# EmbersArc/SCpp

Measured on AMD Instinct MI355X. Metric: converged SCvx trajectories/sec (RocketQuat, K=50) at 1/2/4/8 MI355X, higher is better.
Workload: dtype f64

## Files before the change

### scpp_amd/csrc/common.h

```cpp
#pragma once
#ifdef SCPP_HIP_EMU
#include "hip_emu.h"
#else
#include <hip/hip_runtime.h>
typedef double d4_t __attribute__((ext_vector_type(4)));
#endif
#include <cmath>
#include <cstdint>

namespace scpp
{

constexpr int WAVE = 64;

#ifdef SCPP_HIP_EMU
#define WAVE_SYNC() __syncthreads()
#else
#define WAVE_SYNC()                                            \
    do                                                         \
    {                                                          \
        __builtin_amdgcn_fence(__ATOMIC_ACQ_REL, "wavefront"); \
        __builtin_amdgcn_wave_barrier();                       \
    } while (0)
#endif
// ... 190 lines not shown
__host__ __device__ inline Dual1 dsqrt(Dual1 a)
{
    const double r = sqrt(a.v);
    return Dual1(r, a.d * 0.5 / r);
}
__host__ __device__ inline Dual1 dsin(Dual1 a) { return Dual1(sin(a.v), a.d * cos(a.v)); }
__host__ __device__ inline Dual1 dcos(Dual1 a) { return Dual1(cos(a.v), -a.d * sin(a.v)); }
__host__ __device__ inline double dsqrt(double a) { return sqrt(a); }
__host__ __device__ inline double dsin(double a) { return sin(a); }
__host__ __device__ inline double dcos(double a) { return cos(a); }
__host__ __device__ inline double valueOf(double a) { return a; }
__host__ __device__ inline double valueOf(Dual1 a) { return a.v; }
__host__ __device__ inline double tangentOf(double) { return 0.; }
__host__ __device__ inline double tangentOf(Dual1 a) { return a.d; }

constexpr int RK_S = 13;
constexpr double RK_C[RK_S] = {0., 2. / 27., 1. / 9., 1. / 6., 5. / 12., 1. / 2., 5. / 6., 1. / 6., 2. / 3., 1. / 3., 1., 0., 1.};
constexpr double RK_A[RK_S][RK_S] = {
    {0},
    {2. / 27.},
    {1. / 36., 1. / 12.},
    {1. / 24., 0., 1. / 8.},
    {5. / 12., 0., -25. / 16., 25. / 16.},
    {1. / 20., 0., 0., 1. / 4., 1. / 5.},
    {-25. / 108., 0., 0., 125. / 108., -65. / 27., 125. / 54.},
    {31. / 300., 0., 0., 0., 61. / 225., -2. / 9., 13. / 900.},
    {2., 0., 0., -53. / 6., 704. / 45., -107. / 9., 67. / 90., 3.},
    {-91. / 108., 0., 0., 23. / 108., -976. / 135., 311. / 54., -19. / 60., 17. / 6., -1. / 12.},
    {2383. / 4100., 0., 0., -341. / 164., 4496. / 1025., -301. / 82., 2133. / 4100., 45. / 82., 45. / 164., 18. / 41.},
    {3. / 205., 0., 0., 0., 0., -6. / 41., -3. / 205., -3. / 41., 3. / 41., 6. / 41., 0.},
    {-1777. / 4100., 0., 0., -341. / 164., 4496. / 1025., -289. / 82., 2193. / 4100., 51. / 82., 33. / 164., 12. / 41., 0., 1.}};
constexpr double RK_B[RK_S] = {0., 0., 0., 0., 0., 34. / 105., 9. / 35., 9. / 35., 9. / 280., 9. / 280., 0., 41. / 840., 41. / 840.};

}
```

### scpp_amd/csrc/discretize_kernel.h

```cpp
#pragma once
#include "common.h"
#include <utility>

namespace scpp
{

template <class F, int... S>
__device__ inline void forEachStageImpl(F &&f, std::integer_sequence<int, S...>)
{
    (f(std::integral_constant<int, S>{}), ...);
}
template <class F>
__device__ inline void forEachStage(F &&f)
{
    forEachStageImpl(f, std::make_integer_sequence<int, RK_S>{});
}

#ifndef DISC_STEPS
#define DISC_STEPS 0
#endif
#ifndef DISC_MAX_STEP
#define DISC_MAX_STEP (12. / (14. * 5.))
#endif
constexpr int DISC_STEPS_MAX = 5;
#ifndef DISC_WAVES_PER_SIMD
#define DISC_WAVES_PER_SIMD 2
#endif

template <class Model, bool FOH, bool VT>
struct DiscLayout
{
    static constexpr int NX = Model::NX, NU = Model::NU, NP = Model::NP;
    static constexpr int NJ = NX + NU;
    static constexpr int NCOLS = 1 + NX + NU + (FOH ? NU : 0) + (VT ? 1 : 0);
    static constexpr int NENT = NX * NCOLS;
    static constexpr int NG = WAVE / 16;
    static constexpr int EPL = (NCOLS + NG - 1) / NG;
    static constexpr int COL_S = 1, COL_PHI = 1 + (VT ? 1 : 0), COL_B = COL_PHI + NX, COL_C = COL_B + NU;
    static constexpr int NJP = (NJ + 1) & ~1;
};

template <class Model, bool FOH, bool VT>
struct DiscLds
{
    using L = DiscLayout<Model, FOH, VT>;
    __attribute__((aligned(16))) double Ys[32 * L::NX + 2];
#ifdef DISC_AD_JACOBIAN
    __attribute__((aligned(16))) double Jm[L::NX * L::NJP];
    double fv[L::NX];
    double cst[L::NP + 2 * L::NU + 1];
#else
    double uh[DISC_STEPS_MAX * RK_S * (Model::JacobianRows::NUAUX + 1 + L::NU)];
    __attribute__((aligned(16))) double Wt[Model::JacobianTable::NW];
    double cst[L::NP + 2 * L::NU + Model::JacobianRows::NAUX + 1];
#endif
};

template <class Model, bool FOH, bool VT>
__device__ __forceinline__ void discretizeSegment(int B, int K, const double *__restrict__ X, const double *__restrict__ U,
                                                  const double *__restrict__ sigma, const double *__restrict__ par, int par_stride,
                                                  const int *__restrict__ active, double *__restrict__ Aout, double *__restrict__ Bout,
                                                  double *__restrict__ Cout, double *__restrict__ Sout, double *__restrict__ Zout, int steps_opt,
                                                  const long inst, const int k, DiscLds<Model, FOH, VT> *lds)
{
    using L = DiscLayout<Model, FOH, VT>;
    constexpr int NX = L::NX, NU = L::NU, NP = L::NP, NJ = L::NJ, NJP = L::NJP, NCOLS = L::NCOLS, NG = L::NG, EPL = L::EPL;

    static_assert(NX <= 16 && NCOLS + NG <= 32 && NG == 4, "one 16-row tile of states, two 16-column tiles of V");
    auto &Ys = lds->Ys;
#ifndef DISC_AD_JACOBIAN
    constexpr int NAUX = Model::JacobianRows::NAUX;
    constexpr int NUAUX = Model::JacobianRows::NUAUX;
    constexpr int UHP = NUAUX + 1 + NU;
    auto &uh = lds->uh;
#define DISC_TABLE_ROWS 1
    using TB = typename Model::JacobianTable;
    auto &Wt = lds->Wt;
#else
    constexpr int NAUX = 0;
    auto &Jm = lds->Jm;
    auto &fv = lds->fv;
#endif
    auto &cst = lds->cst;

    const int lane = threadIdx.x;
    for (int i = lane; i < 32 * NX + 2; i += WAVE)
        Ys[i] = 0.;
    const int nseg = K - 1;
    if (inst >= B)
        return;
    if (active && active[inst] == 0)
// ... 99 lines not shown
    const int row = lane & 15, g = lane >> 4;
    const bool lane_on = row < NX;
#ifndef SCPP_HIP_EMU
    __builtin_assume(g >= 0 && g < NG);
#endif
    const double x0r = lane_on ? X[(inst * K + k) * NX + row] : 0.;
    double y[EPL];
    bool eon[EPL];
#pragma unroll
    for (int m = 0; m < EPL; m++)
    {
        const int c = m * NG + g;
        eon[m] = lane_on && c < NCOLS;
        double v = 0.;
        if (c == 0)
            v = x0r;
        else if (c >= L::COL_PHI && c < L::COL_PHI + NX)
            v = (c - L::COL_PHI == row) ? 1. : 0.;
        y[m] = eon[m] ? v : 0.;
    }

    double kk[RK_S][EPL];
    const double h = dt / double(nsteps);
#ifdef DISC_PROFILE
    long long tA = 0, tB = 0, tC = 0;
    const long long tk0 = clock64();
#endif

    for (int step = 0; step < nsteps; step++)
    {
        const double t0 = double(step) * h;
        forEachStage([&](auto sc) {
            constexpr int s = decltype(sc)::value;
#ifdef DISC_PROFILE
            const long long p0 = clock64();
#endif
            const double ts = t0 + RK_C[s] * h;
#pragma unroll
            for (int m = 0; m < EPL; m++)
            {
                double acc = 0.;
#pragma unroll
                for (int j = 0; j < s; j++)
                    if (RK_A[s][j] != 0.)
                        acc += RK_A[s][j] * kk[j][m];
                const double ys = y[m] + h * acc;
                if (eon[m])
                    Ys[(m * NG + g) * NX + row] = ys;
#ifdef DISC_TABLE_ROWS
                if (m == 0 && g == 0 && lane_on)
                    Wt[TB::W_X + row] = ys;
#endif
            }
            WAVE_SYNC();
#ifdef DISC_PROFILE
            const long long p1 = clock64();
            tA += p1 - p0;
#endif
#ifndef DISC_AD_JACOBIAN
            const double frac = FOH ? uh[(step * RK_S + s) * UHP + NUAUX] : 0.;
#else
            const double frac = FOH ? ts / dt : 0.;
#endif
            double jr[NJ];
            double fr;
#ifdef DISC_TABLE_ROWS
// ... 200 lines not shown
            continue;
        Ys[c * NX + row] = y[m];
        if (c >= L::COL_PHI && c < L::COL_PHI + NX)
            Aout[seg * NX * NX + row * NX + (c - L::COL_PHI)] = y[m];
        else if (c >= L::COL_B && c < L::COL_B + NU)
            Bout[seg * NX * NU + row * NU + (c - L::COL_B)] = y[m];
        else if (FOH && c >= L::COL_C && c < L::COL_C + NU)
            Cout[seg * NX * NU + row * NU + (c - L::COL_C)] = y[m];
        else if (VT && c == L::COL_S)
            Sout[seg * NX + row] = y[m];
    }
    if (lane < NX)
        Ys[NCOLS * NX + lane] = x0r;
    WAVE_SYNC();
    if (lane < NX)
    {
        double z = Ys[lane];
#pragma unroll
        for (int j = 0; j < NX; j++)
            z -= Ys[(L::COL_PHI + j) * NX + lane] * Ys[NCOLS * NX + j];
#pragma unroll
        for (int j = 0; j < NU; j++)
        {
            z -= Ys[(L::COL_B + j) * NX + lane] * u0[j];
            if (FOH)
                z -= Ys[(L::COL_C + j) * NX + lane] * u1[j];
        }
        if (VT)
            z -= Ys[L::COL_S * NX + lane] * sg;
        Zout[seg * NX + lane] = z;
    }
}

template <class Model, bool FOH, bool VT>
__global__ void __launch_bounds__(WAVE, DISC_WAVES_PER_SIMD)
    discretize_kernel(int B, int K, const double *__restrict__ X, const double *__restrict__ U,
                      const double *__restrict__ sigma, const double *__restrict__ par, int par_stride,
                      const int *__restrict__ active,
                      double *__restrict__ Aout, double *__restrict__ Bout, double *__restrict__ Cout,
                      double *__restrict__ Sout, double *__restrict__ Zout, int steps_opt)
{
    const int nseg = K - 1;
    const long b = blockIdx.x;
    const long xcd = b & 7, gb = b >> 3;
    const long inst = (gb / nseg) * 8 + xcd;
    const int k = int(gb % nseg);
    __shared__ DiscLds<Model, FOH, VT> lds;
    discretizeSegment<Model, FOH, VT>(B, K, X, U, sigma, par, par_stride, active, Aout, Bout, Cout, Sout, Zout, steps_opt, inst, k, &lds);
}

template <class Model>
__global__ void simulate_kernel(int B, const double *__restrict__ par, int par_stride, const double *__restrict__ dtv,
                                const double *__restrict__ u0v, const double *__restrict__ u1v, double *__restrict__ x,
                                const int *__restrict__ active)
{
    constexpr int NX = Model::NX, NU = Model::NU, NP = Model::NP;
    const long i = long(blockIdx.x) * blockDim.x + threadIdx.x;
    if (i >= B)
        return;
    if (active && active[i] == 0)
        return;
    double p[NP], u0[NU], u1[NU], y[NX], kk[RK_S][NX];
    for (int j = 0; j < NP; j++)
        p[j] = par[i * par_stride + j];
    for (int j = 0; j < NU; j++)
    {
        u0[j] = u0v[i * NU + j];
        u1[j] = u1v[i * NU + j];
    }
    for (int j = 0; j < NX; j++)
        y[j] = x[i * NX + j];
    const double dt = dtv[i];
    const double h = dt / 20.;
    for (int step = 0; step < 20; step++)
    {
        const double t0 = double(step) * h;
#pragma unroll
        for (int s = 0; s < RK_S; s++)
        {
            double ys[NX], u[NU];
            const double ts = t0 + RK_C[s] * h;
            for (int j = 0; j < NX; j++)
            {
                double acc = 0.;
#pragma unroll
                for (int q = 0; q < s; q++)
                    if (RK_A[s][q] != 0.)
                        acc += RK_A[s][q] * kk[q][j];
                ys[j] = y[j] + h * acc;
            }
            for (int j = 0; j < NU; j++)
                u[j] = u0[j] + ts / dt * (u1[j] - u0[j]);
            Model::template systemFlowMap<double>(ys, u, p, kk[s]);
        }
        for (int j = 0; j < NX; j++)
        {
            double acc = 0.;
#pragma unroll
            for (int s = 0; s < RK_S; s++)
                if (RK_B[s] != 0.)
                    acc += RK_B[s] * kk[s][j];
            y[j] += h * acc;
        }
    }
    for (int j = 0; j < NX; j++)
        x[i * NX + j] = y[j];
}

}
```

### scpp_amd/csrc/scpp_hip.cpp

```cpp
#include "../../include/scpp_hip.h"

#include <algorithm>
#include <cmath>
#include <utility>
#include <cstdio>
#include <cstdlib>
#include <cstring>
#include <mutex>
#include <new>
#include <tuple>
#include <vector>

#include "common.h"
#include "discretize_kernel.h"
#include "ipm_solve.h"
#include "ipm_split.h"
#include "model_rocketquat.h"
#include "sc_kernels.h"
#include "scvx_kernels.h"
#include "scvx_persistent.h"
#include "mpc_kernel.h"
#include "mpc_setup.h"

using namespace scpp;

#define CHECK_HIP(expr)                  \
    do                                   \
    {                                    \
        hipError_t e_ = (expr);          \
        if (e_ != hipSuccess)            \
            return SCPP_E_HIP;           \
    } while (0)

template <class L>
struct ParamsOf;
template <class... PL>
struct ParamsOf<PluginList<PL...>>
{
    using type = std::tuple<typename PL::Params...>;
};
template <class F, class... PL>
int withPluginOf(PluginList<PL...>, int model, F &&f)
{
// ... 40 lines not shown
    mpc::MpcConst *mpc_const = nullptr;
    mpc::MpcConst *mpc_host = nullptr;
    double *mpc_xf = nullptr, *mpc_x0 = nullptr, *mpc_U = nullptr, *mpc_X = nullptr, *mpc_cost = nullptr, *mpc_uheld = nullptr, *mpc_t = nullptr;
    int *mpc_status = nullptr, *mpc_iters = nullptr, *mpc_steps = nullptr, *mpc_failed = nullptr, *mpc_ipm = nullptr, *mpc_reached = nullptr;
    bool mpc_ready = false;
    int mpc_B = 0;
    double *sim_dt = nullptr, *sim_u0 = nullptr, *sim_u1 = nullptr, *sim_x = nullptr;
    scpp_sc_opts sc{};
    ParamsOf<Plugins>::type model_params{};
    size_t ws_per = 0;
    scpp_socp_opts socp{1e-8, 1e-7, 1e-7, 60, 1};
    bool sc_ready = false, par_from_ip = false;
    bool sc_warm = false;
    int sc_persistent_min = 3072;
    int mode = SCPP_MODE_FOH | SCPP_MODE_VT;
    struct Span
    {
        hipEvent_t a, b;
        int kind;
        long long inst;
    };
    std::vector<Span> spans;
    std::vector<hipEvent_t> pool;
    scpp_timing timing{};
    hipEvent_t ev_base = nullptr;
    int last_active = 0;
    long long stream_rounds = 0;
    int stream_pools = 0;
    int stream_engine = SCPP_STREAM_ENGINE_DEFAULT;
    double *persist_shares = nullptr;
    unsigned long long stream_ticks[4] = {0, 0, 0, 0};
    int ipm_schedule = SCPP_IPM_SCHEDULE_DEFAULT;
    int ipm_split_pairs = 0;
    int disc_steps = 5;
};

namespace
{

struct DeviceGuard
{
    int prev = -1;
    bool switched = false;
    explicit DeviceGuard(const scpp_hip_ctx *c)
    {
        if (!c)
            return;
        if (hipGetDevice(&prev) == hipSuccess && prev != c->device)
            switched = hipSetDevice(c->device) == hipSuccess;
    }
    ~DeviceGuard()
    {
        if (switched)
            (void)hipSetDevice(prev);
    }
};

template <class T>
int devAlloc(T **p, size_t n)
{
    return hipMalloc(reinterpret_cast<void **>(p), n * sizeof(T)) == hipSuccess ? 0 : -1;
}

hipEvent_t getEvent(scpp_hip_ctx *c)
{
    if (!c->pool.empty())
// ... 88 lines not shown
        else
            c->timing.ms_other += ms;
        if (s.kind == 0 || s.kind == 1)
        {
            if (based)
                iv[s.kind].emplace_back(double(t0), double(t0) + double(ms));
            else
                (s.kind == 0 ? c->timing.ms_discretize_union : c->timing.ms_socp_union) += ms;
        }
        c->pool.push_back(s.a);
        c->pool.push_back(s.b);
    }
    c->timing.ms_discretize_union += unionLength(iv[0]);
    c->timing.ms_socp_union += unionLength(iv[1]);
    c->spans.clear();
}

template <class Model>
int launchDiscretize(scpp_hip_ctx *c, int mode, const double *par0, int stride, const int *active0, long long ninst, Range r)
{
    const int B = r.count, K = c->K;
    const long groups = ((long(B) + 7) / 8) * (K - 1);
    const unsigned grid = unsigned(groups * 8);
    const size_t f = size_t(r.first), nx = size_t(c->nx), nu = size_t(c->nu), seg = size_t(K - 1);
    const double *par = par0 + f * size_t(stride);
    const int *active = active0 ? active0 + f : nullptr;
    struct
    {
        double *X, *U, *sigma, *A, *Bm, *C, *S, *Z;
        hipStream_t stream;
    } v{c->X + f * K * nx, c->U + f * K * nu, c->sigma + f, c->A + f * seg * nx * nx, c->Bm + f * seg * nx * nu,
        c->C + f * seg * nx * nu, c->S + f * seg * nx, c->Z + f * seg * nx, r.stream};
    const bool timed = spanBegin(c, 0, ninst, r.stream);
    if (mode == (SCPP_MODE_FOH | SCPP_MODE_VT))
        hipLaunchKernelGGL((discretize_kernel<Model, true, true>), dim3(grid), dim3(WAVE), 0, v.stream, B, K, v.X, v.U,
                           v.sigma, par, stride, active, v.A, v.Bm, v.C, v.S, v.Z, c->disc_steps);
    else if (mode == SCPP_MODE_FOH)
        hipLaunchKernelGGL((discretize_kernel<Model, true, false>), dim3(grid), dim3(WAVE), 0, v.stream, B, K, v.X, v.U,
                           v.sigma, par, stride, active, v.A, v.Bm, v.C, v.S, v.Z, c->disc_steps);
    else if (mode == SCPP_MODE_VT)
        hipLaunchKernelGGL((discretize_kernel<Model, false, true>), dim3(grid), dim3(WAVE), 0, v.stream, B, K, v.X, v.U,
                           v.sigma, par, stride, active, v.A, v.Bm, v.C, v.S, v.Z, c->disc_steps);
    else
        hipLaunchKernelGGL((discretize_kernel<Model, false, false>), dim3(grid), dim3(WAVE), 0, v.stream, B, K, v.X, v.U,
                           v.sigma, par, stride, active, v.A, v.Bm, v.C, v.S, v.Z, c->disc_steps);
    spanEnd(c, timed, r.stream);
    return hipGetLastError() == hipSuccess ? 0 : SCPP_E_HIP;
}

int discretizeDispatch(scpp_hip_ctx *c, int mode, const double *par, int stride, const int *active, long long ninst, Range r)
{
    return withPlugin(c->model, [&](auto pl) { return launchDiscretize<typename decltype(pl)::Model>(c, mode, par, stride, active, ninst, r); });
}
int discretizeDispatch(scpp_hip_ctx *c, int mode, const double *par, int stride, const int *active, long long ninst)
{
    return discretizeDispatch(c, mode, par, stride, active, ninst, fullRange(c));
}

SCBuffers scBuffers(scpp_hip_ctx *c)
{
    SCBuffers b;
    b.B = c->B;
    b.K = c->K;
    b.x_init_dim = c->x_init;
    b.X = c->X;
    b.U = c->U;
    b.sigma = c->sigma;
    b.ip = c->ip;
    b.uhat = c->uhat;
    b.wtrx = c->wtrx;
    b.active = c->active;
    b.converged = c->converged;
    b.sc_iters = c->sc_iters;
    b.ipm_iters = c->ipm_iters;
    b.status = c->status;
    b.norm1_nu = c->norm1_nu;
    b.sum_delta = c->sum_delta;
    b.delta_sigma = c->delta_sigma;
// ... 243 lines not shown
#if !defined(SCPP_HIP_EMU) && !SCPP_TOOLCHAIN_VALIDATED
    {
        static std::once_flag warned;
        std::call_once(warned, [] {
            std::fprintf(stderr, "scpp_hip: built with an unvalidated toolchain (%s); run `pytest -m gpu` before trusting results\n", scpp_hip_version());
        });
    }
#endif
    int prev_device = -1;
    (void)hipGetDevice(&prev_device);
    CHECK_HIP(hipSetDevice(device_id));
    struct Restore
    {
        int d;
        ~Restore()
        {
            if (d >= 0)
                (void)hipSetDevice(d);
        }
    } restore{prev_device == device_id ? -1 : prev_device};
    if (int rc = tileSelfTest(device_id))
        return rc;
    scpp_hip_ctx *c = new (std::nothrow) scpp_hip_ctx;
    if (!c)
        return SCPP_E_HIP;
    c->device = device_id;
    c->model = model_id;
    c->K = K;
    c->Bmax = batch_max;
    c->B = 0;
    if (const char *e = std::getenv("SCPP_IPM_SCHEDULE"))
        if (std::atoi(e) >= SCPP_IPM_RESIDENT && std::atoi(e) <= SCPP_IPM_SPLIT)
            c->ipm_schedule = std::atoi(e);
    if (const char *e = std::getenv("SCPP_STREAM_ENGINE"))
        if (std::atoi(e) == SCPP_STREAM_POOLS || std::atoi(e) == SCPP_STREAM_PERSISTENT)
            c->stream_engine = std::atoi(e);
    if (const char *e = std::getenv("SCPP_SC_PERSISTENT_MIN"))
        if (std::atoi(e) > 0)
            c->sc_persistent_min = std::atoi(e);
    if (const char *e = std::getenv("SCPP_IPM_SPLIT_PAIRS"))
        if (std::atoi(e) > 0)
            c->ipm_split_pairs = std::atoi(e);
    (void)withPlugin(model_id, [&](auto pl) {
        using PL = decltype(pl);
        c->nx = PL::Model::NX;
        c->nu = PL::Model::NU;
        c->np = PL::Model::NP;
        c->ws_per = ipm::workspaceDoubles<typename PL::Table>(K);
        return 0;
    });
    if (hipStreamCreate(&c->stream) != hipSuccess)
    {
        delete c;
        return SCPP_E_HIP;
    }
    const size_t B = size_t(batch_max), nx = c->nx, nu = c->nu;
    int rc = 0;
    rc |= devAlloc(&c->X, B * K * nx);
    rc |= devAlloc(&c->U, B * K * nu);
    rc |= devAlloc(&c->sigma, B);
    rc |= devAlloc(&c->par, B * c->np);
    rc |= devAlloc(&c->A, B * (K - 1) * nx * nx);
    rc |= devAlloc(&c->Bm, B * (K - 1) * nx * nu);
    rc |= devAlloc(&c->C, B * (K - 1) * nx * nu);
    rc |= devAlloc(&c->S, B * (K - 1) * nx);
    rc |= devAlloc(&c->Z, B * (K - 1) * nx);
// ... 1551 lines not shown
```

### scpp_amd/csrc/scvx_kernels.h

```cpp
#pragma once
#include "discretize_kernel.h"
#include "sc_kernels.h"

namespace scpp
{

constexpr int SCVX_SOLVE_CAP = 64;

struct SCvxBuffers
{
    double *Xold, *Uold;
    double *tr;
    double *last_cost;
    double *cost;
    double *info;
    int *has_last, *needs_disc, *solves;
    double *iter_ring;
    int *iter_count;
    int iter_cap;
};
constexpr int SCVX_ITER_SCALARS = 4;
__host__ __device__ inline size_t scvxIterRecordDoubles(int K, int nx, int nu) { return size_t(K) * size_t(nx + nu) + SCVX_ITER_SCALARS; }
__device__ inline void scvxRecordIterate(const SCBuffers &b, const SCvxBuffers &v, long i, int nx, int nu, int lane, int lanes)
{
// ... 154 lines not shown
#endif
template <class Model>
__device__ __forceinline__ void scvxCostUpdate(const SCBuffers &b, const SCvxBuffers &v, const scpp_scvx_opts &so, const long i)
{
    using namespace ipm;
    constexpr int NX = Model::NX, NU = Model::NU, NP = Model::NP;
    if (i >= b.B || b.active[i] == 0)
        return;
    const int K = b.K, k = threadIdx.x;
    const int foh = so.interpolate_input;
    double acc = 0.;
    if (k < K - 1 && b.status[i] == 0)
    {
        double p[NP], u0[NU], u1[NU], y[NX], kk[RK_S][NX];
        const double *ip = b.ip + i * IP_N;
        for (int j = 0; j < NP; j++)
            p[j] = ip[IP_PAR + j];
        const double *X = b.X + (i * K + k) * NX, *U = b.U + (i * K + k) * NU;
        for (int j = 0; j < NU; j++)
        {
            u0[j] = U[j];
            u1[j] = foh ? U[NU + j] : U[j];
        }
        for (int j = 0; j < NX; j++)
            y[j] = X[j];
        const double dt = b.sigma[i] / double(K - 1);
        const double h = dt / 20.;
        for (int step = 0; step < 20; step++)
        {
            const double t0 = double(step) * h;
#pragma unroll
            for (int s = 0; s < RK_S; s++)
            {
                double ys[NX], u[NU];
                const double ts = t0 + RK_C[s] * h;
                for (int j = 0; j < NX; j++)
                {
                    double a = 0.;
#pragma unroll
                    for (int q = 0; q < s; q++)
                        if (RK_A[s][q] != 0.)
                            a += RK_A[s][q] * kk[q][j];
                    ys[j] = y[j] + h * a;
                }
                for (int j = 0; j < NU; j++)
                    u[j] = u0[j] + ts / dt * (u1[j] - u0[j]);
                Model::template systemFlowMap<double>(ys, u, p, kk[s]);
            }
            for (int j = 0; j < NX; j++)
            {
                double a = 0.;
#pragma unroll
                for (int s = 0; s < RK_S; s++)
                    if (RK_B[s] != 0.)
                        a += RK_B[s] * kk[s][j];
                y[j] += h * a;
            }
        }
        for (int j = 0; j < NX; j++)
            acc += fabs(y[j] - X[NX + j]);
    }
    acc = wave_sum(acc);
    int flags = 0;
    if (k == 0)
    {
        v.cost[i] = acc;
// ... 28 lines not shown
    const int half = lane & 1, pair = lane >> 1;
    const bool solved = b.status[i] == 0;
    if (lane < WAVE)
        seg_sum[lane] = 0.;
    WAVE_SYNC();
    for (int pass = 0; pass * 32 < K - 1; pass++)
    {
        const int k = pass * 32 + pair;
        const bool on = k < K - 1 && solved;
        const int kc = on ? k : 0;
        double p[NP], u0[NU], u1[NU], y[NH], kk[RK_S][NH];
        const double *ip = b.ip + i * IP_N;
#pragma unroll
        for (int j = 0; j < NP; j++)
            p[j] = ip[IP_PAR + j];
        const double *X = b.X + (i * K + kc) * NX, *U = b.U + (i * K + kc) * NU;
#pragma unroll
        for (int j = 0; j < NU; j++)
        {
            u0[j] = U[j];
            u1[j] = foh ? U[NU + j] : U[j];
        }
#pragma unroll
        for (int j = 0; j < NH; j++)
            y[j] = (j < NH1 || !half) ? X[half * NH + j] : 0.;
        const double dt = b.sigma[i] / double(K - 1);
        const double h = dt / 20.;
        for (int step = 0; step < 20; step++)
        {
            const double t0 = double(step) * h;
#pragma unroll
            for (int s = 0; s < RK_S; s++)
            {
                double mine[NH], ys[NX], u[NU], f[NX];
                const double ts = t0 + RK_C[s] * h;
#pragma unroll
                for (int j = 0; j < NH; j++)
                {
                    double a = 0.;
#pragma unroll
                    for (int q = 0; q < s; q++)
                        if (RK_A[s][q] != 0.)
                            a += RK_A[s][q] * kk[q][j];
                    mine[j] = y[j] + h * a;
                }
#pragma unroll
                for (int j = 0; j < NH; j++)
                {
                    const double other = __shfl_xor(mine[j], 1);
                    ys[j] = half ? other : mine[j];
                    if (j < NH1)
                        ys[NH + j] = half ? mine[j] : other;
                }
#pragma unroll
                for (int j = 0; j < NU; j++)
                    u[j] = u0[j] + ts / dt * (u1[j] - u0[j]);
                Model::template systemFlowMap<double>(ys, u, p, f);
#pragma unroll
                for (int j = 0; j < NH; j++)
                    kk[s][j] = half ? (j < NH1 ? f[NH + j < NX ? NH + j : 0] : 0.) : f[j];
            }
#pragma unroll
            for (int j = 0; j < NH; j++)
            {
                double a = 0.;
#pragma unroll
// ... 151 lines not shown
```

### scpp_amd/csrc/scvx_persistent.h

```cpp
#pragma once
#include "discretize_kernel.h"
#include "ipm_solve.h"
#include "scvx_kernels.h"

namespace scpp
{

#ifndef PERSIST_COST_SPLIT
#define PERSIST_COST_SPLIT 1
#endif
struct PersistentOut
{
    double *A, *Bm, *C, *S, *Z;
    int disc_steps;
    double *shares;
};
template <class T>
struct PersistentArgs
{
    ipm::KernelArgs a;
    SCBuffers b;
    SCvxBuffers v;
    StreamQueue q;
    typename T::Params mp;
// ... 72 lines not shown
}
__device__ __forceinline__ int uniformLoad(const int *p)
{
    return uniformInt(*(const volatile int *)p);
}

template <class T>
PERSIST_STEP_FN void persistRefill(long slot)
{
    PERSIST_ARGS(T, A);
    const SCBuffers b = argCopy(A.b);
    const SCvxBuffers v = argCopy(A.v);
    const StreamQueue q = argCopy(A.q);
    const typename T::Params mp = argCopy(A.mp);
    const scpp_sc_opts sc = argCopy(A.sc);
    const scpp_scvx_opts so = argCopy(A.so);
    scvxStreamRefill<T>(b, v, q, mp, sc, so, slot);
    stepFence();
}
template <class T, class Model, bool FOH>
PERSIST_STEP_FN void persistDiscretize(long slot)
{
    PERSIST_ARGS(T, A);
    const int B = A.b.B, K = A.b.K, steps = A.o.disc_steps;
    const double *X = A.a.X, *U = A.a.U, *sigma = A.a.sigma, *par = A.b.ip + ipm::IP_PAR;
    double *Ao = A.o.A, *Bo = A.o.Bm, *Co = A.o.C, *So = A.o.S, *Zo = A.o.Z;
#ifdef SCPP_HIP_EMU
    static DiscLds<Model, FOH, false> lds_obj;
    DiscLds<Model, FOH, false> *lds = &lds_obj;
#else
    extern __shared__ __attribute__((aligned(16))) double seg_lds[];
    DiscLds<Model, FOH, false> *lds = reinterpret_cast<DiscLds<Model, FOH, false> *>(seg_lds);
#endif
    for (int k = 0; k < K - 1; k++)
    {
        discretizeSegment<Model, FOH, false>(B, K, X, U, sigma, par, ipm::IP_N, nullptr, Ao, Bo, Co, So, Zo, steps, slot, k, lds);
        WAVE_SYNC();
    }
    stepFence();
}
template <class T, class P>
PERSIST_STEP_FN void persistSolve(long slot)
{
    PERSIST_ARGS(T, A);
    const ipm::KernelArgs a = argCopy(A.a);
    ipm::ipmSolveInstance<P>(a, int(slot), &A.a);
    if (IPM_PRIO_LANE)
        SET_PRIO(0);
    stepFence();
}
template <class T, class Model>
PERSIST_STEP_FN void persistCost(long slot)
{
    PERSIST_ARGS(T, A);
    const SCBuffers b = argCopy(A.b);
    const SCvxBuffers v = argCopy(A.v);
    const scpp_scvx_opts so = argCopy(A.so);
#if PERSIST_COST_SPLIT
#ifdef SCPP_HIP_EMU
    static double seg_sum[WAVE];
#else
    extern __shared__ __attribute__((aligned(16))) double seg_lds[];
    double *seg_sum = seg_lds;
#endif
    scvxCostUpdateSplit<Model>(b, v, so, slot, seg_sum);
#else
    scvxCostUpdate<Model>(b, v, so, slot);
#endif
    stepFence();
}

// ... 30 lines not shown
        t_disc += t2 - t1;
        t_ipm += t3 - t2;
        t_cost += t4 - t3;
    }
#ifndef SCPP_HIP_EMU
    {
        PERSIST_ARGS(T, A);
        if (A.o.shares && threadIdx.x == 0)
        {
            unsigned long long *sh = reinterpret_cast<unsigned long long *>(A.o.shares);
            atomicAdd(sh + 0, (unsigned long long)t_ref);
            atomicAdd(sh + 1, (unsigned long long)t_disc);
            atomicAdd(sh + 2, (unsigned long long)t_ipm);
            atomicAdd(sh + 3, (unsigned long long)t_cost);
        }
    }
#endif
}

template <class Model, bool FOH, bool VT>
PERSIST_STEP_FN void scPersistDiscretize(long slot)
{
    SC_PERSIST_ARGS(A);
    const int B = A.B, K = A.K, steps = A.disc_steps;
    const double *X = A.a.X, *U = A.a.U, *sigma = A.a.sigma, *par = A.ip + ipm::IP_PAR;
    double *Ao = A.A, *Bo = A.Bm, *Co = A.C, *So = A.S, *Zo = A.Z;
#ifdef SCPP_HIP_EMU
    static DiscLds<Model, FOH, VT> lds_obj;
    DiscLds<Model, FOH, VT> *lds = &lds_obj;
#else
    extern __shared__ __attribute__((aligned(16))) double seg_lds[];
    DiscLds<Model, FOH, VT> *lds = reinterpret_cast<DiscLds<Model, FOH, VT> *>(seg_lds);
#endif
    for (int k = 0; k < K - 1; k++)
    {
        discretizeSegment<Model, FOH, VT>(B, K, X, U, sigma, par, ipm::IP_N, nullptr, Ao, Bo, Co, So, Zo, steps, slot, k, lds);
        WAVE_SYNC();
    }
    stepFence();
}
template <class P>
PERSIST_STEP_FN void scPersistSolve(long slot)
{
    SC_PERSIST_ARGS(A);
    const ipm::KernelArgs a = argCopy(A.a);
    ipm::ipmSolveInstance<P>(a, int(slot), &A.a);
    stepFence();
}
template <class Model, class P, bool FOH, bool VT>
__global__ void __launch_bounds__(WAVE, IPM_WAVES_PER_SIMD) __attribute__((disable_tail_calls)) sc_persistent_kernel(ScPersistentArgs args)
{
#ifdef SCPP_HIP_EMU
    ScPersistentArgsHolder::p = &args;
#else
    if (threadIdx.x == 0)
        persist_kernarg_address = (unsigned long long)__builtin_amdgcn_kernarg_segment_ptr();
    WAVE_SYNC();
#endif
    const long slot = blockIdx.x;
    if (slot >= args.B)
        return;
    const int max_iterations = args.max_iterations;
    for (int it = 0; it < max_iterations; it++)
    {
        SC_PERSIST_ARGS(A);
        if (uniformLoad(A.active + slot) == 0)
            break;
        scPersistDiscretize<Model, FOH, VT>(slot);
        scPersistSolve<P>(slot);
    }
}
// ... 3 lines not shown
```

Baseline: 6189.

## Skip dead RKF78 stage and hoist per-instance setup out of segment loop

Adds a constexpr liveness test for the 13 RK stages and skips any stage whose weight and later dependents are all zero. For RKF78 with 8th-order weights that is stage 10, removing one Jacobian evaluation per step. Adds a new segment body that hoists per-instance setup (LDS zeroing, parameter prep, Jacobian-table slot coefficients) out of the per-segment loop. It also double-buffers the stage state in LDS (Ys/Ys1) to drop a barrier between stages. Costs extra LDS and more registers for the cached table slots, which may reduce occupancy; an env var restores the old path.

```diff
diff --git a/scpp_amd/csrc/common.h b/scpp_amd/csrc/common.h
--- a/scpp_amd/csrc/common.h
+++ b/scpp_amd/csrc/common.h
@@ -246,4 +246,25 @@
     {-1777. / 4100., 0., 0., -341. / 164., 4496. / 1025., -289. / 82., 2193. / 4100., 51. / 82., 33. / 164., 12. / 41., 0., 1.}};
 constexpr double RK_B[RK_S] = {0., 0., 0., 0., 0., 34. / 105., 9. / 35., 9. / 35., 9. / 280., 9. / 280., 0., 41. / 840., 41. / 840.};
 
-}
+#ifndef RK_SKIP_DEAD
+#define RK_SKIP_DEAD 1
+#endif
+constexpr bool rkStageLive(int s)
+{
+    if (RK_B[s] != 0.)
+        return true;
+    for (int r = s + 1; r < RK_S; r++)
+        if (RK_A[r][s] != 0.)
+            return true;
+    return false;
+}
+constexpr int rkLiveBefore(int s)
+{
+    int n = 0;
+    for (int j = 0; j < s; j++)
+        n += rkStageLive(j) ? 1 : 0;
+    return n;
+}
+static_assert(rkLiveBefore(RK_S) == RK_S - 1 && !rkStageLive(10), "RKF78 with the 8th-order weights: exactly one dead stage, index 10");
+
+}
diff --git a/scpp_amd/csrc/discretize_kernel.h b/scpp_amd/csrc/discretize_kernel.h
--- a/scpp_amd/csrc/discretize_kernel.h
+++ b/scpp_amd/csrc/discretize_kernel.h
@@ -25,6 +25,14 @@
 constexpr int DISC_STEPS_MAX = 5;
 #ifndef DISC_WAVES_PER_SIMD
 #define DISC_WAVES_PER_SIMD 2
+#endif
+
+#ifndef DISC_STAGE_SCHEDULE
+#define DISC_STAGE_SCHEDULE 1
+#endif
+#ifdef DISC_AD_JACOBIAN
+#undef DISC_STAGE_SCHEDULE
+#define DISC_STAGE_SCHEDULE 0
 #endif
 
 template <class Model, bool FOH, bool VT>
@@ -45,6 +53,9 @@
 {
     using L = DiscLayout<Model, FOH, VT>;
     __attribute__((aligned(16))) double Ys[32 * L::NX + 2];
+#if DISC_STAGE_SCHEDULE
+    __attribute__((aligned(16))) double Ys1[32 * L::NX + 2];
+#endif
 #ifdef DISC_AD_JACOBIAN
     __attribute__((aligned(16))) double Jm[L::NX * L::NJP];
     double fv[L::NX];
@@ -56,7 +67,7 @@
 #endif
 };
 
-template <class Model, bool FOH, bool VT>
+template <class Model, bool FOH, bool VT, bool SKIP = (RK_SKIP_DEAD != 0)>
 __device__ __forceinline__ void discretizeSegment(int B, int K, const double *__restrict__ X, const double *__restrict__ U,
                                                   const double *__restrict__ sigma, const double *__restrict__ par, int par_stride,
                                                   const int *__restrict__ active, double *__restrict__ Aout, double *__restrict__ Bout,
@@ -222,6 +233,8 @@
         const double t0 = double(step) * h;
         forEachStage([&](auto sc) {
             constexpr int s = decltype(sc)::value;
+            if (SKIP && !rkStageLive(s))
+                return;
 #ifdef DISC_PROFILE
             const long long p0 = clock64();
 #endif
@@ -488,7 +501,364 @@
     }
 }
 
+#if DISC_STAGE_SCHEDULE
+template <class Model>
+struct DiscTableSlots
+{
+    using TB = typename Model::JacobianTable;
+    double tcf[2][TB::MAXMON];
+    unsigned tof[2][TB::MAXMON][2];
+    int ttg[2];
+};
+
 template <class Model, bool FOH, bool VT>
+__device__ __forceinline__ bool discretizeSetup(int B, const double *__restrict__ par, int par_stride, const int *__restrict__ active, const long inst,
+                                                DiscLds<Model, FOH, VT> *lds, DiscTableSlots<Model> &ts)
+{
+    using L = DiscLayout<Model, FOH, VT>;
+    using TB = typename Model::JacobianTable;
+    constexpr int NX = L::NX, NU = L::NU, NP = L::NP, NAUX = Model::JacobianRows::NAUX;
+    static_assert(NX <= 16 && L::NCOLS + L::NG <= 32 && L::NG == 4, "one 16-row tile of states, two 16-column tiles of V");
+    const int lane = threadIdx.x;
+    if (inst >= B)
+        return false;
+    if (active && active[inst] == 0)
+        return false;
+    for (int i = lane; i < 32 * NX + 2; i += WAVE)
+    {
+        lds->Ys[i] = 0.;
+        lds->Ys1[i] = 0.;
+    }
+    for (int i = lane; i < TB::NW; i += WAVE)
+        lds->Wt[i] = (i == TB::W_ONE) ? 1. : 0.;
+    WAVE_SYNC();
+    if (lane == 0)
+    {
+        double p[NP], aux0[NAUX];
+#pragma unroll
+        for (int i = 0; i < NP; i++)
+            p[i] = par[inst * par_stride + i];
+        Model::JacobianRows::prepare(p, aux0);
+#pragma unroll
+        for (int i = 0; i < NP; i++)
+        {
+            lds->cst[i] = p[i];
+            lds->Wt[TB::W_PAR + i] = p[i];
+        }
+#pragma unroll
+        for (int i = 0; i < NAUX; i++)
+        {
+            lds->cst[NP + 2 * NU + i] = aux0[i];
+            lds->Wt[TB::W_AUX + i] = aux0[i];
+        }
+    }
+#pragma unroll
+    for (int ps = 0; ps < 2; ps++)
+    {
+        const int slot = ps * 64 + lane;
+        ts.ttg[ps] = TB::target(slot);
+#pragma unroll
+        for (int q = 0; q < TB::MAXMON; q++)
+        {
+            ts.tcf[ps][q] = TB::coef(slot, q);
+            ts.tof[ps][q][0] = unsigned(TB::factor(slot, q, 0) * 8) | (unsigned(TB::factor(slot, q, 1) * 8) << 16);
+            ts.tof[ps][q][1] = unsigned(TB::factor(slot, q, 2) * 8) | (unsigned(TB::factor(slot, q, 3) * 8) << 16);
+        }
+    }
+    WAVE_SYNC();
+    return true;
+}
+
+template <class Model, bool FOH, bool VT, bool SKIP>
+__device__ __forceinline__ void discretizeSegmentBody(int K, const double *__restrict__ X, const double *__restrict__ U, const double *__restrict__ sigma,
+                                                      double *__restrict__ Aout, double *__restrict__ Bout, double *__restrict__ Cout,
+                                                      double *__restrict__ Sout, double *__restrict__ Zout, int steps_opt, const long inst, const int k,
+                                                      DiscLds<Model, FOH, VT> *lds, const DiscTableSlots<Model> &ts)
+{
+    using L = DiscLayout<Model, FOH, VT>;
+    using TB = typename Model::JacobianTable;
+    constexpr int NX = L::NX, NU = L::NU, NP = L::NP, NJ = L::NJ, NCOLS = L::NCOLS, NG = L::NG, EPL = L::EPL;
+    constexpr int NAUX = Model::JacobianRows::NAUX, NUAUX = Model::JacobianRows::NUAUX, UHP = NUAUX + 1 + NU;
+    constexpr int NLIVE = SKIP ? rkLiveBefore(RK_S) : RK_S;
+    auto &Ys = lds->Ys;
+    auto &uh = lds->uh;
+    auto &Wt = lds->Wt;
+    auto &cst = lds->cst;
+    (void)NAUX;
+
+    const int lane = threadIdx.x;
+    const int nseg = K - 1;
+    const double sg = sigma[inst];
+    const double dt = VT ? 1. / double(K - 1) : sg / double(K - 1);
+    const double tscale = VT ? sg : 1.;
+    int nsteps = DISC_STEPS > 0 ? DISC_STEPS : steps_opt;
+    if (nsteps <= 0)
+    {
+        const double seg_seconds = fabs(sg) / double(K - 1);
+        nsteps = int(ceil(seg_seconds / DISC_MAX_STEP));
+        nsteps = nsteps < 1 ? 1 : (nsteps > DISC_STEPS_MAX ? DISC_STEPS_MAX : nsteps);
+    }
+    nsteps = uniformInt(nsteps);
+    double u0[NU], u1[NU];
+#pragma unroll
+    for (int i = 0; i < NU; i++)
+    {
+        u0[i] = U[(inst * K + k) * NU + i];
+        u1[i] = FOH ? U[(inst * K + k + 1) * NU + i] : u0[i];
+    }
+    if (lane == 0)
+    {
+#pragma unroll
+        for (int i = 0; i < NU; i++)
+        {
+            cst[NP + i] = u0[i];
+            cst[NP + NU + i] = u1[i];
+        }
+    }
+    {
+        double p[NP];
+#pragma unroll
+        for (int i = 0; i < NP; i++)
+            p[i] = cst[i];
+        const double hh = dt / double(nsteps);
+        for (int e = lane; e < nsteps * RK_S; e += WAVE)
+        {
+            const double tse = double(e / RK_S) * hh + RK_C[e % RK_S] * hh;
+            const double fre = FOH ? tse / dt : 0.;
+            double ue[NU], ua[NUAUX];
+#pragma unroll
+            for (int i = 0; i < NU; i++)
+                ue[i] = u0[i] + fre * (u1[i] - u0[i]);
+            Model::JacobianRows::prepareInput(ue, p, ua);
+#pragma unroll
+            for (int i = 0; i < NUAUX; i++)
+                uh[e * UHP + i] = ua[i];
+            uh[e * UHP + NUAUX] = fre;
+#pragma unroll
+            for (int i = 0; i < NU; i++)
+                uh[e * UHP + NUAUX + 1 + i] = ue[i];
+        }
+    }
+    WAVE_SYNC();
+
+    const int row = lane & 15, g = lane >> 4;
+    const bool lane_on = row < NX;
+#ifndef SCPP_HIP_EMU
+    __builtin_assume(g >= 0 && g < NG);
+#endif
+    const double x0r = lane_on ? X[(inst * K + k) * NX + row] : 0.;
+    double y[EPL];
+    bool eon[EPL];
+#pragma unroll
+    for (int m = 0; m < EPL; m++)
+    {
+        const int c = m * NG + g;
+        eon[m] = lane_on && c < NCOLS;
+        double v = 0.;
+        if (c == 0)
+            v = x0r;
+        else if (c >= L::COL_PHI && c < L::COL_PHI + NX)
+            v = (c - L::COL_PHI == row) ? 1. : 0.;
+        y[m] = eon[m] ? v : 0.;
+    }
+
+    double kk[RK_S][EPL];
+    const double h = dt / double(nsteps);
+    for (int step = 0; step < nsteps; step++)
+    {
+        forEachStage([&](auto sc) {
+            constexpr int s = decltype(sc)::value;
+            if (SKIP && !rkStageLive(s))
+                return;
+            constexpr int ord = SKIP ? rkLiveBefore(s) : s;
+            const int buf = (NLIVE % 2 == 0) ? (ord & 1) : ((ord + step) & 1);
+            double *Yb = buf ? lds->Ys1 : lds->Ys;
+            const int e = step * RK_S + s;
+            double ys0 = 0.;
+#pragma unroll
+            for (int m = 0; m < EPL; m++)
+            {
+                double acc = 0.;
+#pragma unroll
+                for (int j = 0; j < s; j++)
+                    if (RK_A[s][j] != 0.)
+                        acc += RK_A[s][j] * kk[j][m];
+                const double ys = y[m] + h * acc;
+                if (eon[m])
+                    Yb[(m * NG + g) * NX + row] = ys;
+                if (m == 0)
+                {
+                    ys0 = ys;
+                    if (g == 0 && lane_on)
+                        Wt[TB::W_X + row] = ys;
+                }
+            }
+            {
+                double xs[NX], hh[TB::NH];
+#pragma unroll
+                for (int i = 0; i < NX; i++)
+                    xs[i] = readLane(ys0, i);
+                TB::evalHoists(xs, uh + e * UHP + NUAUX + 1, cst, cst + NP + 2 * NU, uh + e * UHP, hh);
+                if (lane == 0)
+                {
+#pragma unroll
+                    for (int i = 0; i < TB::NH; i++)
+                        Wt[TB::W_H + i] = hh[i];
+                }
+                if (lane < NU)
+                    Wt[TB::W_U + lane] = uh[e * UHP + NUAUX + 1 + lane];
+                else if (lane < NU + NUAUX)
+                    Wt[TB::W_UAUX + lane - NU] = uh[e * UHP + lane - NU];
+            }
+            WAVE_SYNC();
+            const double frac = FOH ? uh[e * UHP + NUAUX] : 0.;
+            const char *wb = reinterpret_cast<const char *>(Wt);
+#pragma unroll
+            for (int ps = 0; ps < 2; ps++)
+            {
+                double val = 0.;
+#pragma unroll
+                for (int q = 0; q < (ps == 0 ? TB::MAXMON : TB::MAXMON_B); q++)
+                {
+                    const double f0 = *reinterpret_cast<const double *>(wb + (ts.tof[ps][q][0] & 0xFFFFu));
+                    const double f1 = *reinterpret_cast<const double *>(wb + (ts.tof[ps][q][0] >> 16));
+                    const double f2 = *reinterpret_cast<const double *>(wb + (ts.tof[ps][q][1] & 0xFFFFu));
+                    const double f3 = *reinterpret_cast<const double *>(wb + (ts.tof[ps][q][1] >> 16));
+                    val += ((ts.tcf[ps][q] * f0) * f1) * (f2 * f3);
+                }
+                if (ts.ttg[ps] >= 0)
+                    Wt[ts.ttg[ps]] = val;
+                WAVE_SYNC();
+            }
+            const int rowc = lane_on ? row : 0;
+            double bsel[4];
+#pragma unroll
+            for (int t = 0; t < 4; t++)
+            {
+                const double v = Wt[TB::W_J + rowc * NJ + (4 * t + g < NX ? 4 * t + g : 0)];
+                bsel[t] = (4 * t + g < NX) ? v : 0.;
+            }
+            const double fr = Wt[TB::W_F + rowc];
+            const double alphaB = FOH ? (1. - frac) : 1.;
+            d4_t acc0 = {0., 0., 0., 0.}, acc1 = {0., 0., 0., 0.};
+#pragma unroll
+            for (int t = 0; t < 4; t++)
+            {
+                const int kx = g + 4 * t;
+                const double b = bsel[t] * tscale;
+                acc0 = __builtin_amdgcn_mfma_f64_16x16x4f64(Yb[row * NX + kx], b, acc0, 0, 0, 0);
+                if (NCOLS > 16)
+                    acc1 = __builtin_amdgcn_mfma_f64_16x16x4f64(Yb[(16 + row) * NX + kx], b, acc1, 0, 0, 0);
+            }
+#pragma unroll
+            for (int m = 0; m < EPL; m++)
+            {
+                const int c = m * NG + g;
+                const double acc = m < 4 ? acc0[m < 4 ? m : 0] : acc1[m >= 4 ? m - 4 : 0];
+                double d = acc;
+                const bool slotB = m * NG < L::COL_B + NU && m * NG + NG > L::COL_B;
+                const bool slotC = FOH && m * NG < L::COL_C + NU && m * NG + NG > L::COL_C;
+                if (slotB || slotC)
+                {
+                    const bool isB = c >= L::COL_B && c < L::COL_B + NU;
+                    const bool isC = FOH && c >= L::COL_C && c < L::COL_C + NU;
+                    const int jj = isB ? c - L::COL_B : isC ? c - L::COL_C : 0;
+                    const double w = isB ? alphaB : isC ? frac : 0.;
+                    const double jb = Wt[TB::W_J + rowc * NJ + NX + jj];
+                    d += (w * tscale) * jb;
+                }
+                if (VT && m * NG <= L::COL_S && m * NG + NG > L::COL_S)
+                    d = (c == L::COL_S) ? d + fr : d;
+                if (m == 0)
+                    d = (c == 0) ? tscale * fr : d;
+                kk[s][m] = d;
+            }
+        });
+#pragma unroll
+        for (int m = 0; m < EPL; m++)
+        {
+            double acc = 0.;
+#pragma unroll
+            for (int s = 0; s < RK_S; s++)
+                if (RK_B[s] != 0.)
+                    acc += RK_B[s] * kk[s][m];
+            y[m] += h * acc;
+        }
+    }
+    WAVE_SYNC();
+
+    const long seg = inst * nseg + k;
+#pragma unroll
+    for (int m = 0; m < EPL; m++)
+    {
+        const int c = m * NG + g;
+        if (!eon[m])
+            continue;
+        Ys[c * NX + row] = y[m];
+        if (c >= L::COL_PHI && c < L::COL_PHI + NX)
+            Aout[seg * NX * NX + row * NX + (c - L::COL_PHI)] = y[m];
+        else if (c >= L::COL_B && c < L::COL_B + NU)
+            Bout[seg * NX * NU + row * NU + (c - L::COL_B)] = y[m];
+        else if (FOH && c >= L::COL_C && c < L::COL_C + NU)
+            Cout[seg * NX * NU + row * NU + (c - L::COL_C)] = y[m];
+        else if (VT && c == L::COL_S)
+            Sout[seg * NX + row] = y[m];
+    }
+    if (lane < NX)
+        Ys[NCOLS * NX + lane] = x0r;
+    WAVE_SYNC();
+    if (lane < NX)
+    {
+        double z = Ys[lane];
+#pragma unroll
+        for (int j = 0; j < NX; j++)
+            z -= Ys[(L::COL_PHI + j) * NX + lane] * Ys[NCOLS * NX + j];
+#pragma unroll
+        for (int j = 0; j < NU; j++)
+        {
+            z -= Ys[(L::COL_B + j) * NX + lane] * u0[j];
+            if (FOH)
+                z -= Ys[(L::COL_C + j) * NX + lane] * u1[j];
+        }
+        if (VT)
+            z -= Ys[L::COL_S * NX + lane] * sg;
+        Zout[seg * NX + lane] = z;
+    }
+    WAVE_SYNC();
+    if (lane < NX)
+        Ys[NCOLS * NX + lane] = 0.;
+    WAVE_SYNC();
+}
+#endif
+
+template <class Model, bool FOH, bool VT, int SCHED = DISC_STAGE_SCHEDULE, bool SKIP = (RK_SKIP_DEAD != 0)>
+__device__ __forceinline__ void discretizeSegments(int B, int K, const double *__restrict__ X, const double *__restrict__ U,
+                                                   const double *__restrict__ sigma, const double *__restrict__ par, int par_stride,
+                                                   const int *__restrict__ active, double *__restrict__ Aout, double *__restrict__ Bout,
+                                                   double *__restrict__ Cout, double *__restrict__ Sout, double *__restrict__ Zout, int steps_opt,
+                                                   const long inst, const int k0, const int k1, DiscLds<Model, FOH, VT> *lds)
+{
+#if DISC_STAGE_SCHEDULE
+    if constexpr (SCHED != 0)
+    {
+        DiscTableSlots<Model> ts;
+        if (!discretizeSetup<Model, FOH, VT>(B, par, par_stride, active, inst, lds, ts))
+            return;
+        for (int k = k0; k < k1; k++)
+            discretizeSegmentBody<Model, FOH, VT, SKIP>(K, X, U, sigma, Aout, Bout, Cout, Sout, Zout, steps_opt, inst, k, lds, ts);
+    }
+    else
+#endif
+    {
+        for (int k = k0; k < k1; k++)
+        {
+            discretizeSegment<Model, FOH, VT, SKIP>(B, K, X, U, sigma, par, par_stride, active, Aout, Bout, Cout, Sout, Zout, steps_opt, inst, k, lds);
+            WAVE_SYNC();
+        }
+    }
+}
+
+template <class Model, bool FOH, bool VT, int SCHED = DISC_STAGE_SCHEDULE, bool SKIP = (RK_SKIP_DEAD != 0)>
 __global__ void __launch_bounds__(WAVE, DISC_WAVES_PER_SIMD)
     discretize_kernel(int B, int K, const double *__restrict__ X, const double *__restrict__ U,
                       const double *__restrict__ sigma, const double *__restrict__ par, int par_stride,
@@ -502,7 +872,7 @@
     const long inst = (gb / nseg) * 8 + xcd;
     const int k = int(gb % nseg);
     __shared__ DiscLds<Model, FOH, VT> lds;
-    discretizeSegment<Model, FOH, VT>(B, K, X, U, sigma, par, par_stride, active, Aout, Bout, Cout, Sout, Zout, steps_opt, inst, k, &lds);
+    discretizeSegments<Model, FOH, VT, SCHED, SKIP>(B, K, X, U, sigma, par, par_stride, active, Aout, Bout, Cout, Sout, Zout, steps_opt, inst, k, k + 1, &lds);
 }
 
 template <class Model>
@@ -534,6 +904,8 @@
 #pragma unroll
         for (int s = 0; s < RK_S; s++)
         {
+            if (RK_SKIP_DEAD && !rkStageLive(s))
+                continue;
             double ys[NX], u[NU];
             const double ts = t0 + RK_C[s] * h;
             for (int j = 0; j < NX; j++)
diff --git a/scpp_amd/csrc/scpp_hip.cpp b/scpp_amd/csrc/scpp_hip.cpp
--- a/scpp_amd/csrc/scpp_hip.cpp
+++ b/scpp_amd/csrc/scpp_hip.cpp
@@ -9,6 +9,7 @@
 #include <mutex>
 #include <new>
 #include <tuple>
+#include <type_traits>
 #include <vector>
 
 #include "common.h"
@@ -115,6 +116,7 @@
     unsigned long long stream_ticks[4] = {0, 0, 0, 0};
     int ipm_schedule = SCPP_IPM_SCHEDULE_DEFAULT;
     int ipm_split_pairs = 0;
+    int disc_schedule = DISC_STAGE_SCHEDULE;
     int disc_steps = 5;
 };
 
@@ -269,18 +271,26 @@
     } v{c->X + f * K * nx, c->U + f * K * nu, c->sigma + f, c->A + f * seg * nx * nx, c->Bm + f * seg * nx * nu,
         c->C + f * seg * nx * nu, c->S + f * seg * nx, c->Z + f * seg * nx, r.stream};
     const bool timed = spanBegin(c, 0, ninst, r.stream);
-    if (mode == (SCPP_MODE_FOH | SCPP_MODE_VT))
-        hipLaunchKernelGGL((discretize_kernel<Model, true, true>), dim3(grid), dim3(WAVE), 0, v.stream, B, K, v.X, v.U,
-                           v.sigma, par, stride, active, v.A, v.Bm, v.C, v.S, v.Z, c->disc_steps);
-    else if (mode == SCPP_MODE_FOH)
-        hipLaunchKernelGGL((discretize_kernel<Model, true, false>), dim3(grid), dim3(WAVE), 0, v.stream, B, K, v.X, v.U,
-                           v.sigma, par, stride, active, v.A, v.Bm, v.C, v.S, v.Z, c->disc_steps);
-    else if (mode == SCPP_MODE_VT)
-        hipLaunchKernelGGL((discretize_kernel<Model, false, true>), dim3(grid), dim3(WAVE), 0, v.stream, B, K, v.X, v.U,
-                           v.sigma, par, stride, active, v.A, v.Bm, v.C, v.S, v.Z, c->disc_steps);
+    auto launch = [&](auto foh, auto vt, auto old) {
+        constexpr int SCHED = decltype(old)::value ? 0 : DISC_STAGE_SCHEDULE;
+        constexpr bool SKIP = decltype(old)::value ? false : (RK_SKIP_DEAD != 0);
+        hipLaunchKernelGGL((discretize_kernel<Model, decltype(foh)::value, decltype(vt)::value, SCHED, SKIP>), dim3(grid), dim3(WAVE), 0, v.stream, B, K,
+                           v.X, v.U, v.sigma, par, stride, active, v.A, v.Bm, v.C, v.S, v.Z, c->disc_steps);
+    };
+    auto launchMode = [&](auto old) {
+        if (mode == (SCPP_MODE_FOH | SCPP_MODE_VT))
+            launch(std::true_type{}, std::true_type{}, old);
+        else if (mode == SCPP_MODE_FOH)
+            launch(std::true_type{}, std::false_type{}, old);
+        else if (mode == SCPP_MODE_VT)
+            launch(std::false_type{}, std::true_type{}, old);
+        else
+            launch(std::false_type{}, std::false_type{}, old);
+    };
+    if (c->disc_schedule == 0 && (DISC_STAGE_SCHEDULE != 0 || RK_SKIP_DEAD != 0))
+        launchMode(std::true_type{});
     else
-        hipLaunchKernelGGL((discretize_kernel<Model, false, false>), dim3(grid), dim3(WAVE), 0, v.stream, B, K, v.X, v.U,
-                           v.sigma, par, stride, active, v.A, v.Bm, v.C, v.S, v.Z, c->disc_steps);
+        launchMode(std::false_type{});
     spanEnd(c, timed, r.stream);
     return hipGetLastError() == hipSuccess ? 0 : SCPP_E_HIP;
 }
@@ -590,6 +600,9 @@
     if (const char *e = std::getenv("SCPP_IPM_SCHEDULE"))
         if (std::atoi(e) >= SCPP_IPM_RESIDENT && std::atoi(e) <= SCPP_IPM_SPLIT)
             c->ipm_schedule = std::atoi(e);
+    if (const char *e = std::getenv("SCPP_DISC_SCHEDULE"))
+        if (std::atoi(e) == 0)
+            c->disc_schedule = 0;
     if (const char *e = std::getenv("SCPP_STREAM_ENGINE"))
         if (std::atoi(e) == SCPP_STREAM_POOLS || std::atoi(e) == SCPP_STREAM_PERSISTENT)
             c->stream_engine = std::atoi(e);
diff --git a/scpp_amd/csrc/scvx_kernels.h b/scpp_amd/csrc/scvx_kernels.h
--- a/scpp_amd/csrc/scvx_kernels.h
+++ b/scpp_amd/csrc/scvx_kernels.h
@@ -210,6 +210,8 @@
 #pragma unroll
             for (int s = 0; s < RK_S; s++)
             {
+                if (RK_SKIP_DEAD && !rkStageLive(s))
+                    continue;
                 double ys[NX], u[NU];
                 const double ts = t0 + RK_C[s] * h;
                 for (int j = 0; j < NX; j++)
@@ -304,6 +306,8 @@
 #pragma unroll
             for (int s = 0; s < RK_S; s++)
             {
+                if (RK_SKIP_DEAD && !rkStageLive(s))
+                    continue;
                 double mine[NH], ys[NX], u[NU], f[NX];
                 const double ts = t0 + RK_C[s] * h;
 #pragma unroll
diff --git a/scpp_amd/csrc/scvx_persistent.h b/scpp_amd/csrc/scvx_persistent.h
--- a/scpp_amd/csrc/scvx_persistent.h
+++ b/scpp_amd/csrc/scvx_persistent.h
@@ -128,11 +128,7 @@
     extern __shared__ __attribute__((aligned(16))) double seg_lds[];
     DiscLds<Model, FOH, false> *lds = reinterpret_cast<DiscLds<Model, FOH, false> *>(seg_lds);
 #endif
-    for (int k = 0; k < K - 1; k++)
-    {
-        discretizeSegment<Model, FOH, false>(B, K, X, U, sigma, par, ipm::IP_N, nullptr, Ao, Bo, Co, So, Zo, steps, slot, k, lds);
-        WAVE_SYNC();
-    }
+    discretizeSegments<Model, FOH, false>(B, K, X, U, sigma, par, ipm::IP_N, nullptr, Ao, Bo, Co, So, Zo, steps, slot, 0, K - 1, lds);
     stepFence();
 }
 template <class T, class P>
@@ -229,11 +225,7 @@
     extern __shared__ __attribute__((aligned(16))) double seg_lds[];
     DiscLds<Model, FOH, VT> *lds = reinterpret_cast<DiscLds<Model, FOH, VT> *>(seg_lds);
 #endif
-    for (int k = 0; k < K - 1; k++)
-    {
-        discretizeSegment<Model, FOH, VT>(B, K, X, U, sigma, par, ipm::IP_N, nullptr, Ao, Bo, Co, So, Zo, steps, slot, k, lds);
-        WAVE_SYNC();
-    }
+    discretizeSegments<Model, FOH, VT>(B, K, X, U, sigma, par, ipm::IP_N, nullptr, Ao, Bo, Co, So, Zo, steps, slot, 0, K - 1, lds);
     stepFence();
 }
 template <class P>
```

Result: faster. 6294 (median of 6 runs) (+1.7%).
